# RapidAI/RapidDoc

Hardware: AMD Instinct MI355X
Metric: pages/sec (layout+OCR det/rec) (higher is better)
Workload: dtype f32

## Files before the change

### rapiddoc_amd/_lib.py

```python
from __future__ import annotations

import ctypes as C
from pathlib import Path

_PKG = Path(__file__).resolve().parent
LIB_PATH = _PKG / "librapiddoc_mi355.so"
_lib = None

SYMBOLS = {
    "rd_version": (C.c_char_p, []),
    "rd_create": (C.c_void_p, [C.c_int, C.c_char_p]),
    "rd_create_error": (C.c_char_p, []),
    "rd_destroy": (None, [C.c_void_p]),
    "rd_last_error": (C.c_char_p, [C.c_void_p]),
    "rd_load_weights": (C.c_int, [C.c_void_p, C.c_void_p, C.c_size_t]),
    "rd_query_workspace": (C.c_int, [C.c_void_p, C.c_int, C.c_int, C.c_int, C.c_int, C.POINTER(C.c_size_t)]),
    "rd_det_forward": (C.c_int, [C.c_void_p, C.c_void_p, C.c_int, C.c_int, C.c_int, C.c_void_p, C.c_void_p, C.c_size_t, C.c_void_p]),
    "rd_det_forward_ex": (C.c_int, [C.c_void_p, C.c_void_p, C.c_int, C.c_int, C.c_int, C.c_void_p, C.c_int, C.c_void_p, C.c_void_p, C.c_size_t, C.c_void_p]),
    "rd_rec_forward": (C.c_int, [C.c_void_p, C.c_void_p, C.c_int, C.c_int, C.c_void_p, C.c_void_p, C.c_void_p, C.c_int, C.c_void_p, C.c_size_t, C.c_void_p]),
    "rd_rec_num_classes": (C.c_int, [C.c_void_p]),
    "rd_rec_token_dim": (C.c_int, [C.c_void_p]),
    "rd_rec_backbone_forward": (C.c_int, [C.c_void_p, C.c_void_p, C.c_int, C.c_int, C.c_void_p, C.c_void_p, C.c_size_t, C.c_void_p]),
    "rd_rec_backbone_forward_lines": (C.c_int, [C.c_void_p, C.c_void_p, C.c_int, C.c_int, C.c_void_p, C.c_void_p, C.c_void_p, C.c_size_t, C.c_void_p]),
    "rd_rec_tail_forward": (C.c_int, [C.c_void_p, C.c_void_p, C.c_int, C.c_int, C.c_int, C.c_void_p, C.c_void_p, C.c_void_p, C.c_void_p,
# ... 3 lines not shown
    "rd_formula_encoder_forward": (C.c_int, [C.c_void_p, C.c_void_p, C.c_int, C.c_int, C.c_int, C.c_int, C.c_void_p, C.c_void_p, C.c_size_t, C.c_void_p]),
    "rd_formula_decode": (C.c_int, [C.c_void_p, C.c_void_p, C.c_int, C.c_int, C.c_int, C.c_void_p, C.POINTER(C.c_int32), C.c_void_p]),
    "rd_formula_decode_stream": (C.c_int, [C.c_void_p, C.c_void_p, C.c_int, C.c_int, C.c_int, C.c_int, C.c_void_p, C.c_void_p, C.c_void_p, C.c_void_p]),
    "rd_formula_max_new_tokens": (C.c_int, [C.c_void_p]),
    "rd_preproc_resize_norm": (C.c_int, [C.c_int, C.c_void_p, C.c_int, C.c_int, C.c_int, C.c_int, C.POINTER(C.c_float), C.POINTER(C.c_float), C.c_float, C.c_int, C.c_int, C.c_void_p, C.c_void_p]),
    "rd_preproc_resize_norm_batch": (C.c_int, [C.c_int, C.c_void_p, C.c_int, C.c_int, C.c_int, C.c_int, C.c_int, C.POINTER(C.c_float), C.POINTER(C.c_float), C.c_float, C.c_int, C.c_int, C.c_void_p, C.c_void_p]),
    "rd_preproc_resize_aa_norm": (C.c_int, [C.c_int, C.c_void_p, C.c_int, C.c_int, C.c_int, C.c_int, C.POINTER(C.c_float), C.POINTER(C.c_float), C.c_int, C.c_void_p, C.c_void_p, C.c_void_p]),
    "rd_formula_margin_boxes": (C.c_int, [C.c_int, C.c_void_p, C.c_int, C.c_void_p, C.c_void_p]),
    "rd_formula_preproc_plan": (C.c_int, [C.c_int, C.c_int, C.c_void_p]),
    "rd_formula_preproc_batch": (C.c_int, [C.c_int, C.c_void_p, C.c_void_p, C.c_int, C.c_void_p, C.c_void_p, C.c_void_p]),
    "rd_crop_resize_norm_batch": (C.c_int, [C.c_int, C.c_void_p, C.c_int, C.c_int, C.c_int, C.c_void_p, C.c_int, C.c_int, C.c_int, C.POINTER(C.c_float), C.POINTER(C.c_float), C.c_float, C.c_int, C.c_void_p, C.c_void_p]),
    "rd_line_crops_batch": (C.c_int, [C.c_int, C.c_void_p, C.c_int, C.c_int, C.c_int, C.c_void_p, C.c_int, C.c_int64, C.c_void_p, C.c_int, C.c_int, C.c_int, C.c_void_p, C.c_void_p]),
    "rd_line_warp_batch": (C.c_int, [C.c_int, C.c_void_p, C.c_int, C.c_int, C.c_int, C.c_void_p, C.c_int, C.c_int64, C.c_void_p, C.c_void_p]),
    "rd_line_resize_norm_batch": (C.c_int, [C.c_int, C.c_void_p, C.c_int, C.c_void_p, C.c_int, C.c_int, C.c_int, C.c_void_p, C.c_void_p]),
    "rd_cls_forward": (C.c_int, [C.c_void_p, C.c_void_p, C.c_int, C.c_int, C.c_int, C.c_void_p, C.c_int, C.c_void_p, C.c_void_p, C.c_size_t, C.c_void_p]),
    "rd_table_encoder_forward": (C.c_int, [C.c_void_p, C.c_void_p, C.c_int, C.c_int, C.c_int, C.c_void_p, C.c_void_p, C.c_size_t, C.c_void_p]),
    "rd_table_decode": (C.c_int, [C.c_void_p, C.c_void_p, C.c_int, C.c_int, C.c_int, C.c_void_p, C.c_void_p, C.c_void_p, C.c_void_p]),
    "rd_table_decode_stream": (C.c_int, [C.c_void_p, C.c_void_p, C.c_int, C.c_int, C.c_int, C.c_int, C.c_void_p, C.c_void_p, C.c_void_p, C.c_void_p, C.c_void_p]),
    "rd_line_flip180_batch": (C.c_int, [C.c_int, C.c_void_p, C.c_int, C.c_void_p, C.c_float, C.c_void_p, C.c_void_p, C.c_void_p]),
    "rd_ctc_collapse": (C.c_int, [C.c_int, C.c_void_p, C.c_void_p, C.c_int, C.c_int, C.c_void_p, C.c_int, C.c_int, C.c_void_p, C.c_int, C.c_void_p]),
    "rd_ctc_collapse_lines": (C.c_int, [C.c_int, C.c_void_p, C.c_void_p, C.c_int, C.c_void_p, C.c_int, C.c_void_p, C.c_int, C.c_int, C.c_void_p, C.c_int, C.c_void_p, C.c_void_p,
                                        C.c_void_p]),
    "rd_db_postprocess": (C.c_int, [C.c_void_p, C.c_int, C.c_int, C.c_int, C.c_void_p, C.c_float, C.c_float, C.c_float, C.c_int, C.c_int, C.c_void_p, C.c_int, C.c_void_p, C.c_int]),
    "rd_db_boxes_workspace": (C.c_size_t, [C.c_int, C.c_int, C.c_int, C.c_int, C.c_int]),
    "rd_db_boxes_device": (C.c_int, [C.c_int, C.c_void_p, C.c_int, C.c_int, C.c_int, C.c_void_p, C.c_float, C.c_float, C.c_float, C.c_int, C.c_int,
                                     C.c_int, C.c_void_p, C.c_size_t, C.c_void_p, C.c_int, C.c_void_p, C.c_void_p]),
    "rd_rec_chunk_cost": (C.c_double, [C.c_int, C.c_int, C.c_int]),
    "rd_rec_plan_chunks": (C.c_int, [C.c_void_p, C.c_int, C.c_int, C.c_int, C.c_int, C.c_int, C.c_void_p, C.c_int, C.c_void_p]),
    "rd_rec_plan_lines": (C.c_int, [C.c_void_p, C.c_void_p] + [C.c_int] * 9 + [C.c_void_p] * 4 + [C.c_int, C.c_void_p]),
    "rd_text_boxes_order_merge": (C.c_int, [C.c_void_p, C.c_void_p, C.c_int, C.c_int, C.c_void_p, C.c_void_p]),
    "rd_ctc_rows_text": (C.c_int, [C.c_void_p, C.c_int, C.c_int, C.c_void_p, C.c_int64, C.c_void_p, C.c_void_p, C.c_void_p, C.c_void_p]),
    "rd_layout_postprocess": (C.c_int, [C.c_void_p, C.c_int, C.c_int, C.c_int, C.c_int, C.c_void_p, C.c_void_p, C.c_void_p, C.c_void_p]),
    "rd_layout_postprocess_select": (C.c_int, [C.c_void_p, C.c_int, C.c_int, C.c_int, C.c_int, C.c_void_p, C.c_void_p, C.c_void_p, C.c_void_p]),
    "rd_find_external_contours": (C.c_int, [C.c_void_p, C.c_int, C.c_int, C.c_void_p, C.c_int, C.c_void_p, C.c_int, C.c_void_p, C.c_void_p]),
    "rd_find_external_contours_none": (C.c_int, [C.c_void_p, C.c_int, C.c_int, C.c_void_p, C.c_int, C.c_void_p, C.c_int, C.c_void_p, C.c_void_p]),
    "rd_checkbox_workspace": (C.c_size_t, [C.c_int, C.c_int, C.c_int, C.c_int, C.c_int, C.c_void_p]),
    "rd_checkbox_detect_device": (C.c_int, [C.c_int, C.c_void_p, C.c_int, C.c_int, C.c_int, C.c_int, C.c_int, C.c_int, C.c_void_p, C.c_size_t, C.c_void_p,
                                            C.c_void_p, C.c_void_p]),
    "rd_checkbox_finish": (C.c_int, [C.c_void_p, C.c_int, C.c_int, C.c_int, C.c_void_p, C.c_int, C.c_void_p]),
    "rd_region_canvases_workspace": (C.c_size_t, [C.c_int, C.c_int, C.c_int]),
    "rd_region_canvases": (C.c_int, [C.c_int, C.c_void_p, C.c_int, C.c_void_p, C.c_void_p, C.c_int, C.c_int, C.c_void_p, C.c_void_p, C.c_void_p, C.c_size_t,
                                     C.c_void_p]),
    "rd_stage_pack": (C.c_int, [C.c_void_p, C.c_void_p, C.c_void_p, C.c_void_p, C.c_void_p, C.c_int, C.c_void_p, C.c_int64, C.c_int]),
    "rd_stage_canvases": (C.c_int, [C.c_int, C.c_void_p, C.c_void_p, C.c_int, C.c_void_p]),
    "rd_contour_area": (C.c_double, [C.c_void_p, C.c_int]),
    "rd_arc_length": (C.c_double, [C.c_void_p, C.c_int, C.c_int]),
    "rd_approx_poly_dp": (C.c_int, [C.c_void_p, C.c_int, C.c_double, C.c_int, C.c_void_p, C.c_void_p]),
    "rd_min_area_rect_points": (C.c_int, [C.c_void_p, C.c_int, C.c_void_p]),
    "rd_polygon_area": (C.c_double, [C.c_void_p, C.c_int]),
    "rd_polygon_intersection_area": (C.c_double, [C.c_void_p, C.c_int, C.c_void_p, C.c_int]),
    "rd_fill_poly": (C.c_int, [C.c_void_p, C.c_int, C.c_int, C.c_void_p, C.c_int, C.c_int]),
    "rd_msdeform_attn": (C.c_int, [C.c_int] + [C.c_void_p] * 6 + [C.c_int] * 7 + [C.c_void_p]),
    "rd_topk_rows": (C.c_int, [C.c_int, C.c_void_p, C.c_int, C.c_int, C.c_int, C.c_void_p, C.c_void_p, C.c_void_p]),
    "rd_encoder_layer_workspace": (C.c_size_t, [C.c_int, C.c_int, C.c_int]),
    "rd_encoder_layer": (C.c_int, [C.c_int, C.c_void_p, C.c_void_p] + [C.c_int] * 6 + [C.c_void_p] * 12 + [C.c_float, C.c_void_p, C.c_void_p, C.c_size_t, C.c_void_p]),
    "rd_set_precision": (C.c_int, [C.c_void_p, C.c_char_p]),
    "rd_range_status": (C.c_int, [C.c_void_p, C.c_void_p]),
    "rd_plan_stats": (C.c_int, [C.c_void_p, C.POINTER(C.c_uint64), C.POINTER(C.c_uint64), C.POINTER(C.c_uint64)]),
    "rd_set_profiling": (C.c_int, [C.c_void_p, C.c_int]),
    "rd_profile_json": (C.c_char_p, [C.c_void_p]),
}

_I, _P, _F = C.c_int, C.c_void_p, C.c_float
DEBUG_SYMBOLS = {
    "rd_debug_det_forward_stages": (_I, [_P, _P, _I, _I, _I, _P, _P, _P]),
    "rd_debug_cls_forward_stages": (_I, [_P, _P, _I, _I, _I, _P, _P, _P, _P]),
    "rd_debug_table_decode": (_I, [_P, _P, _I, _I, _I, _P] + [_P] * 7),
    "rd_debug_table_decode_stream": (_I, [_P, _P, _I, _I, _I, _I, _P, _P, _P, _P, _P, _P, _P, _P, _I]),
    "rd_debug_table_encoder_taps": (_I, [_P, _P, _I, _I, _I, _P, _P, _P]),
    "rd_debug_formula_decode": (_I, [_P, _P, _I, _I, _I, _P, C.POINTER(C.c_int32), _P, _P, _P]),
    "rd_debug_formula_decode_stream": (_I, [_P, _P, _I, _I, _I, _I, _P, _P, _P, _P, _P, _P, _P, _I]),
    "rd_debug_resize_aa_coeffs": (_I, [_I, _I, _P, _P, C.c_int64]),
    "rd_debug_resample_coeffs": (_I, [_I, _I, C.c_double, C.c_double, _I, _P, _P, C.c_int64]),
    "rd_debug_region_keep_mask": (_I, [_I, _I, _P, _I, _P]),
    "rd_debug_time_mixer": (_F, [_I] * 4 + [_P] * 6),
    "rd_debug_time_gemm": (_F, [_I] * 5 + [_P] * 6),
    "rd_debug_gemm_h1": (_F, [_I] * 5 + [_P, _I, _P, _P, _P, _I, _P, _I, _P]),
    "rd_debug_seqconv": (_F, [_I] * 8 + [_P, _I, _P, _I, _P, _P, _P, _P, _I, _P]),
    "rd_debug_det_local": (_F, [_I] * 5 + [_P] * 5 + [_F, _P, C.POINTER(C.c_int)]),
    "rd_debug_conv_route": (_I, [_I] * 17 + [_P, _I]),
    "rd_debug_conv_ex": (_F, [_I] * 22 + [_P] * 10 + [C.c_char_p, _P, _I, _P]),
    "rd_debug_conv": (_F, [_I] * 14 + [_P] * 8),
    "rd_debug_stem34": (_F, [_I] * 11 + [_P] * 7),
    "rd_debug_dwconv_ex": (_F, [_I] * 17 + [_P] * 10 + [_I]),
    "rd_debug_dwconv": (_F, [_I] * 8 + [_P] * 8),
    "rd_debug_dw_route": (_I, [_I] * 9 + [_P, _I, _P]),
    "rd_debug_weight_split": (_I, [_P, _I, _I, _P, _P]),
    "rd_debug_lcv3_dw": (_F, [_I] * 9 + [_P] * 8),
    "rd_debug_dw5_strip": (_F, [_I] * 11 + [_P] * 7),
    "rd_debug_mv1e_pool": (_I, [_I] * 4 + [_P] * 3),
    "rd_debug_derived_tensor": (C.c_long, [C.c_char_p, C.c_char_p, C.c_size_t, C.c_char_p, _P, C.c_long]),
    "rd_debug_mbv3_dw": (_F, [_I] * 12 + [_P] * 4),
    "rd_debug_mbv3_block": (_F, [_I] * 14 + [_P] * 8),
    "rd_debug_mbv3_block_ok": (_I, [_I] * 12),
    "rd_debug_mbv3s_dw": (_F, [_I] * 13 + [_P] * 4),
    "rd_debug_mbv3s_block": (_F, [_I] * 15 + [_P] * 12),
    "rd_debug_lcv3_dw_det": (_F, [_I] * 10 + [_P] * 5),
    "rd_debug_lcv3_block": (_F, [_I] * 9 + [_P] * 9),
    "rd_debug_time_ctc": (_F, [_I] * 4 + [_P] * 7 + [_I, _P]),
    "rd_debug_time_checkbox_mask": (_F, [_I] * 4 + [_P, _P]),
    "rd_debug_attention": (_I, [_I] * 4 + [_F, _P, _P, _P, _I, _P]),
    "rd_debug_vit_attention": (_I, [_I] * 4 + [_F, _P, _P]),
    "rd_debug_attention_limits": (_I, [_I, _P, _P]),
    "rd_debug_layernorm": (_I, [_I, _I, _P, _I, _P, _I, _P, _P, _F]),
    "rd_debug_se_chain": (_I, [_I] * 7 + [_F] + [_I] * 3 + [_P] * 9),
    "rd_debug_maxpool2x2s1": (_I, [_I] * 6 + [_P] * 2),
    "rd_debug_avgpool3x2": (_I, [_I] * 6 + [_P] * 3),
    "rd_debug_mask_cols": (_I, [_I] * 5 + [_P, _P, _I]),
    "rd_debug_upsample": (_I, [_I] * 8 + [_P] * 2),
    "rd_debug_add": (_I, [_I] * 5 + [_P] * 3),
    "rd_debug_det_head_tail": (_I, [_I] * 4 + [_P] * 6),
    "rd_debug_ctc_head": (_I, [_I] * 3 + [_P, _I] + [_P] * 6 + [_I, _P, _P]),
    "rd_debug_dec_gemv": (_I, [_I] * 4 + [_P] * 7),
    "rd_debug_dec_attention": (_I, [_I] * 4 + [_P, _P, _I, C.c_longlong] + [_P] * 5 + [_P, _I, _P, _P, _I, _P, _I]),
    "rd_debug_dec_select": (_I, [_I, _P, _I, _I, _I, _P, _I, _P, _I, _I] + [_P] * 6),
    "rd_debug_td_gemv": (_I, [_I] * 4 + [_P] * 5),
    "rd_debug_td_attention": (_I, [_I] * 4 + [_P, _P, _I, C.c_longlong, _P, _I, _P, _P, _I, _P, _I, _P, _P]),
    "rd_debug_td_select": (_I, [_I, _P, _I, _P, _I, _P, _I, _P, _P, _P, _I, _P, _P, _P, _P, _I] + [_P] * 6),
}


class NativeLibraryError(RuntimeError):
    pass


def load():
    global _lib
    if _lib is not None:
        return _lib
    if not LIB_PATH.exists():
        raise NativeLibraryError(
            f"{LIB_PATH} is missing - build it with `python -m rapiddoc_amd.build` (hipcc, gfx950). "
            "rapiddoc_amd has no CPU fallback.")
    import torch
    lib = C.CDLL(str(LIB_PATH))
    for name, (res, args) in {**SYMBOLS, **DEBUG_SYMBOLS}.items():
        fn = getattr(lib, name)
        fn.restype = res
        fn.argtypes = args
    _lib = lib
    return lib
```

### rapiddoc_amd/csrc/api_debug.cpp

```cpp
#include <algorithm>
#include <cstring>
#include <functional>
#include <string>
#include <vector>

#include "api_handle.h"
#include "builder_util.h"
#include "region_geom.h"

extern "C" {

static float rd_debug_time(int iters, const std::function<void()>& launch, const std::function<void()>& after_first = nullptr) {
    hipEvent_t e0, e1;
    (void)hipEventCreate(&e0); (void)hipEventCreate(&e1);
    launch();
    if (after_first) after_first();
    (void)hipEventRecord(e0, nullptr);
    for (int i = 0; i < iters; ++i) launch();
    (void)hipEventRecord(e1, nullptr);
    (void)hipEventSynchronize(e1);
    float ms = 0.f;
    (void)hipEventElapsedTime(&ms, e0, e1);
    (void)hipEventDestroy(e0); (void)hipEventDestroy(e1);
    return iters > 0 ? ms / iters : 0.f;
// ... 425 lines not shown
        if ((images & 8) && !deconv && rd::conv9x9_h1_shape_ok(KH, KW, Cin, Cout)) {
            p.w9_inv = rd::prepare_conv9x9_h1_weights(hw.data(), Cout, Cin, img);
            d = nullptr;
            if (!upload(img, &d)) return done(-1.f);
            p.w9 = (const uint16_t*)d;
        }
        if (range_out) {
            if (hipHostMalloc((void**)&flag, sizeof(unsigned), hipHostMallocMapped) != hipSuccess) { flag = nullptr; return done(-1.f); }
            *flag = 0;
            p.range_flag = flag;
        }
    } else if (range_out) {
        *range_out = 0;
    }
    rd::ConvRoute route = split ? rd::conv_split_route(p, ascale != nullptr) : rd::conv_f32_route(p);
    if (force) {
        if (!debug_conv_tile(force, split, &route)) return done(-1.f);
        if (split && ((unsigned long long)N * H * W * (unsigned long long)xld >= (1ull << 32) ||
                      (unsigned long long)p.Ng * (unsigned long long)((p.K + 31) & ~31) >= (1ull << 32)))
            return done(-1.f);
    }
    if (old && split && old->code == 2 && rd::conv_stream_h3_supported(p)) route = rd::CONV_STREAM;
    else if (old && split && old->code == 1 && rd::conv_direct_h3_supported(p)) route = rd::CONV_DIRECT;
    if (ln_g && route != rd::CONV_SKINNY) return done(-1.f);
    if (route_out) *route_out = route;
    float ms = -2.f;
    try {
        ms = rd_debug_time(iters, [&] { rd::launch_conv_route(route, p, nullptr); });
    } catch (const std::exception&) {
        ms = -2.f;
    }
    return done(ms);
}

float rd_debug_conv_ex(int N, int H, int W, int Cin, int Cout, int KH, int KW, int SH, int SW, int PT, int PL, int PB, int PR, int act, int xld, int yld,
                       int rld, int out_mode, int split, int images, int allow_skinny, int iters, float* x, float* w, float* bias, float* res, float* y,
                       const float* dscale, const float* dshift, const float* ln_g, const float* ln_b, const float* ascale, const char* force,
                       char* name, int name_len, int* range_out) {
    rd::ConvRoute route = rd::CONV_F32_128x128;
    debug_copy_name("", name, name_len);
    const float ms = debug_conv_run(N, H, W, Cin, Cout, KH, KW, SH, SW, PT, PL, PB, PR, act, xld, yld, rld, out_mode, split, images, allow_skinny, iters,
                                    x, w, bias, res, y, dscale, dshift, ln_g, ln_b, ascale, force, nullptr, &route, range_out);
    if (ms != -1.f) debug_copy_name(rd::conv_route_name(route), name, name_len);
    return ms;
}

float rd_debug_conv(int N, int H, int W, int Cin, int Cout, int KH, int KW, int S, int PT, int PL, int PB, int PR, int act, int iters,
                    float* x, float* w, void* wh, void* wl, float* bias, float* res, float* y, int* used_direct) {
    const DebugConvOld old{wh, wl, used_direct ? *used_direct : 0};
    const int images = old.code == 0 ? 4 : old.code == 4 ? 8 : 0;
    rd::ConvRoute route = rd::CONV_F32_128x128;
    const float ms = debug_conv_run(N, H, W, Cin, Cout, KH, KW, S, S, PT, PL, PB, PR, act, Cin, Cout, Cout, rd::OUT_NHWC, wh != nullptr, images, 0, iters, x,
                                    w, bias, res, y, nullptr, nullptr, nullptr, nullptr, nullptr, nullptr, &old, &route, nullptr);
    if (used_direct && ms != -1.f) *used_direct = debug_conv_code(route);
    return ms;
}

float rd_debug_stem34(int N, int H, int W, int Cin, int xld, int N1, int N2, int yld, int act3, int act4, int iters, float* x, float* w3, float* b3,
                      float* w4, float* b4, float* y, unsigned* range_flag) {
    if (!rd::stem34_shape_ok(Cin, N1, N2)) return -1.f;
    std::vector<float> h3((size_t)N1 * 9 * Cin), h4((size_t)N2 * N1), hb3((size_t)((N1 + 31) / 32) * 32, 0.f);
    if (hipMemcpy(h3.data(), w3, h3.size() * 4, hipMemcpyDeviceToHost) != hipSuccess) return -1.f;
    if (hipMemcpy(h4.data(), w4, h4.size() * 4, hipMemcpyDeviceToHost) != hipSuccess) return -1.f;
    if (hipMemcpy(hb3.data(), b3, (size_t)N1 * 4, hipMemcpyDeviceToHost) != hipSuccess) return -1.f;
    std::vector<uint16_t> i3, i4;
    float inv[2];
    rd::prepare_stem34_weights(h3.data(), h4.data(), Cin, N1, N2, i3, i4, inv);
    void *d3 = nullptr, *d4 = nullptr, *db3 = nullptr;
    if (hipMalloc(&d3, i3.size() * 2) != hipSuccess || hipMalloc(&d4, i4.size() * 2) != hipSuccess || hipMalloc(&db3, hb3.size() * 4) != hipSuccess) return -1.f;
    (void)hipMemcpy(d3, i3.data(), i3.size() * 2, hipMemcpyHostToDevice);
    (void)hipMemcpy(d4, i4.data(), i4.size() * 2, hipMemcpyHostToDevice);
    (void)hipMemcpy(db3, hb3.data(), hb3.size() * 4, hipMemcpyHostToDevice);
    rd::Stem34Params p{};
    p.x = x; p.xld = xld; p.N = N; p.H = H; p.W = W; p.Cin = Cin; p.y = y; p.yld = yld;
    p.OH = (H - 1) / 2 + 1; p.OW = (W - 1) / 2 + 1; p.N1 = N1; p.N2 = N2;
    p.w3 = (const uint16_t*)d3; p.w3_inv = inv[0]; p.b3 = (const float*)db3;
    p.w4 = (const uint16_t*)d4; p.w4_inv = inv[1]; p.b4 = b4;
    p.act3 = act3; p.act4 = act4; p.range_flag = range_flag;
    const float ms = rd_debug_time(iters, [&] { rd::launch_stem34(p, nullptr); });
    (void)hipFree(d3); (void)hipFree(d4); (void)hipFree(db3);
    return ms;
}

static std::string debug_dw_route_name(const rd::DwRoute& r) {
    static const char* const kernels[] = {"pixel", "lds", "kxk_lds", "col", "tiled"};
    return std::string(kernels[r.kernel]) + (r.kernel == rd::DW_PIXEL || r.kernel == rd::DW_COL ? "" : std::to_string(r.variant));
}

float rd_debug_dwconv_ex(int N, int H, int W, int C, int KH, int KW, int SH, int SW, int PT, int PL, int PB, int PR, int act, int xld, int yld, int rld,
                         int iters, float* x, float* w, float* bias, float* res, float* y, const int32_t* line_w, const int32_t* tokinfo, float* gap,
                         int* gap_chunks, char* name, int name_len) {
    if (N <= 0 || H <= 0 || W <= 0 || C <= 0 || C % 4 != 0 || KH <= 0 || KW <= 0 || SH <= 0 || SW <= 0 || PT < 0 || PL < 0 || PB < 0 || PR < 0) return -1.f;
    if (!x || !w || !y || xld < C || xld % 4 != 0 || yld < C || yld % 4 != 0 || (res && (rld < C || rld % 4 != 0))) return -1.f;
    if (H + PT + PB < KH || W + PL + PR < KW) return -1.f;
    rd::DwParams p = rd::dw_geometry(N, H, W, C, KH, KW, SH, SW, PT, PL, PB, PR);
    if (tokinfo && !(N == 1 && H == 1 && KH == 1 && SW == 1 && p.OW == W)) return -1.f;
    if (line_w && !(SW == 1 && p.OW == W)) return -1.f;
    p.x = x; p.xld = xld; p.w = w; p.bias = bias; p.y = y; p.yld = yld; p.act = act; p.res = res; p.rld = res ? rld : 0;
    p.tokinfo = tokinfo;
    if (line_w) { p.line_w = line_w; p.line_w_stride = 1; }
    p.gap_chunks = rd::dwconv_gap_chunks(p);
    p.gap_partial = p.gap_chunks > 0 ? gap : nullptr;
    const rd::DwRoute r = rd::dw_route(p, p.gap_partial != nullptr);
    if (gap_chunks) *gap_chunks = r.kernel == rd::DW_KXK_LDS ? -1 : p.gap_chunks;
    debug_copy_name(debug_dw_route_name(r).c_str(), name, name_len);
    return rd_debug_time(iters, [&] { rd::launch_dwconv(p, nullptr); });
}

float rd_debug_dwconv(int N, int H, int W, int C, int K, int SH, int act, int iters, float* x, float* w, float* bias, float* res, float* y,
                      const int32_t* line_w, float* gap, int* gap_chunks) {
    return rd_debug_dwconv_ex(N, H, W, C, K, K, SH, 1, K / 2, K / 2, K / 2, K - 1 - K / 2, act, C, C, C, iters, x, w, bias, res, y, line_w, nullptr, gap,
                              gap_chunks, nullptr, 0);
}

int rd_debug_dw_route(int N, int H, int W, int C, int K, int SH, int ragged, int has_line_w, int wants_gap, char* name, int name_len, int* gap_chunks) {
    if (N <= 0 || H <= 0 || W <= 0 || C <= 0 || K <= 0 || SH <= 0) return -1;
    static const int32_t table[1] = {};
    rd::DwParams p{};
    p.xld = p.yld = p.rld = C; p.N = N; p.H = H; p.W = W; p.C = C;
    p.KH = ragged ? 1 : K; p.KW = ragged ? 3 : K; p.SH = SH; p.SW = 1; p.PT = p.KH / 2; p.PL = p.KW / 2;
    p.OH = (H + 2 * p.PT - p.KH) / SH + 1; p.OW = W;
    const int planned = rd::dwconv_gap_chunks(p);
    if (ragged) p.tokinfo = table;
    if (has_line_w) { p.line_w = table; p.line_w_stride = 1; }
    const rd::DwRoute r = rd::dw_route(p, wants_gap != 0);
    debug_copy_name(debug_dw_route_name(r).c_str(), name, name_len);
    if (gap_chunks) *gap_chunks = r.gap_chunks;
    return planned;
}

int rd_debug_weight_split(const float* w, int n, int clamp, uint16_t* scaled, uint16_t* h3) {
    if (!w || n <= 0 || !scaled || !h3) return -1000;
    const int ex = rd::rd_pow2_exp(w, (size_t)n, clamp);
    for (int i = 0; i < n; ++i) {
        rd::rd_split_scaled(w[i], ex, scaled[2 * i], scaled[2 * i + 1]);
        rd::rd_split_2048(w[i], h3[2 * i], h3[2 * i + 1]);
    }
    return ex;
}

float rd_debug_lcv3_dw(int N, int H, int W, int C, int K, int SH, int SW, int pre_act, int iters, const float* aff, float* x, float* w, float* bias,
                       float* y, const int32_t* line_in, const int32_t* line_out, float* gap) {
    if (!rd::lcv3_dw_shape_ok(K, SH, SW, C) || !aff || (gap && !rd::lcv3_gap_shape_ok(C))) return -1.f;
    rd::Lcv3DwParams p{};
    p.x = x; p.xld = C; p.N = N; p.H = H; p.W = W; p.C = C; p.w = w; p.bias = bias; p.y = y; p.yld = C;
    p.K = K; p.SH = SH; p.SW = SW;
    p.OH = (H + 2 * (K / 2) - K) / SH + 1; p.OW = (W + 2 * (K / 2) - K) / SW + 1;
    p.pre_act = pre_act; p.pre_s = aff[0]; p.pre_b = aff[1]; p.post_s = aff[2]; p.post_b = aff[3]; p.post_act = 1;
    p.line_in = line_in; p.line_out = line_out; p.line_stride = 1;
    return rd_debug_time(iters, [&] { rd::launch_lcv3_dw(p, nullptr); },
                         [&] { if (gap) rd::launch_lcv3_gap_rows(y, C, N, p.OH, p.OW, C, gap, line_out, 1, nullptr); });
}

float rd_debug_dw5_strip(int N, int H, int W, int C, int SH, int SW, int pre_act, int post_act, int xld, int yld, int iters, const float* aff, float* x,
                         float* w, float* bias, float* y, const int32_t* line_in, const int32_t* line_out) {
    if (!aff || SH < 1 || SW < 1) return -1.f;
    rd::Lcv3DwParams p{};
    p.x = x; p.xld = xld; p.N = N; p.H = H; p.W = W; p.C = C; p.w = w; p.bias = bias; p.y = y; p.yld = yld;
    p.K = 5; p.SH = SH; p.SW = SW;
    p.OH = (H - 1) / SH + 1; p.OW = (W - 1) / SW + 1;
    p.pre_act = pre_act; p.pre_s = aff[0]; p.pre_b = aff[1]; p.post_s = aff[2]; p.post_b = aff[3]; p.post_act = post_act;
    p.line_in = line_in; p.line_out = line_out; p.line_stride = 1;
    if (!rd::dw5_strip_launch_ok(p)) return -1.f;
    return rd_debug_time(iters, [&] { (void)rd::launch_dw5_strip(p, nullptr); });
}

// ... 330 lines not shown
```

### rapiddoc_amd/csrc/kernels_stem_fused.hip

```cpp
#include <cmath>
#include <cstdlib>
#include <vector>

#include "rd_device.h"

namespace rd {

static constexpr int SF_TH = 8, SF_TW = 32;
static constexpr int SF_EH = SF_TH + 2, SF_EW = SF_TW + 2;
static constexpr int SF_AH = SF_TH + 1, SF_AW = SF_TW + 1;
static constexpr int SF_PH = 2 * SF_EH + 1, SF_PW = 2 * SF_EW + 1;
static constexpr int SF_PROW = 208;
static constexpr int SF_PATCH_FLOATS = SF_PH * SF_PROW + 16;
static constexpr int SF_NT = 512;

template <int C1>
struct SfGeom {
    static constexpr int CA = C1, NA = C1 / 2, CB = (NA + 7) / 8 * 8;
    static constexpr int K1 = 48, K2A = 4 * CA, K2B = 4 * CB;
    static constexpr int SE = CA + 4, SA = CB + 4;
    static_assert(((SE / 4) & 1) == 1 && ((SA / 4) & 1) == 1, "pixel strides must be 4 x odd floats");
    static constexpr int pad8(int k) { return ((k / 8) & 1) ? k : k + 8; }
    static constexpr int R1 = pad8(K1), R2A = pad8(K2A), R2B = pad8(K2B);
    static constexpr int W1_H = C1 * R1, W2A_H = NA * R2A, W2B_H = C1 * R2B;
// ... 4 lines not shown
    static constexpr int A_FLOATS_RAW = (SF_AH * SF_AW + 31) / 32 * 32 * SA;
    static constexpr int A_FLOATS = A_FLOATS_RAW > SF_PATCH_FLOATS ? A_FLOATS_RAW : SF_PATCH_FLOATS;
    static constexpr size_t LDS_BYTES = (size_t)W_HALFS * 2 + (size_t)(BIAS_FLOATS + E_FLOATS + A_FLOATS) * 4 + 64;
    static constexpr int MB1 = (SF_EH * SF_EW + 31) / 32, NB1 = (C1 + 31) / 32;
    static constexpr int MB2 = (SF_AH * SF_AW + 31) / 32;
    static constexpr int MB3 = SF_TH * SF_TW / 32, NB3 = (C1 + 31) / 32;
    static_assert(NA <= 32 && MB3 == 8, "one N block for stem2a, one M block per wavefront for stem2b");
};

struct StemFusedParams {
    const float* x; int N, H, W, in_ch;
    const uint16_t* wimg;
    const float* bias;
    float* y; int yld;
    int H2, W2, tiles_x, tiles_y;
    unsigned* range_flag;
    const int32_t* line_tab;
    int dbg;
};

typedef _Float16 sf_f16x2 __attribute__((ext_vector_type(2)));
__device__ __forceinline__ void sf_split8(const f32x4 a, const f32x4 b, float neg1, f16x8& hi, f16x8& lo) {
#pragma unroll
    for (int e = 0; e < 4; e += 2) {
        const sf_f16x2 ha = __builtin_convertvector(f32x2{a[e], a[e + 1]}, sf_f16x2);
        const sf_f16x2 hb = __builtin_convertvector(f32x2{b[e], b[e + 1]}, sf_f16x2);
        hi[e] = ha[0];
        hi[e + 1] = ha[1];
        hi[4 + e] = hb[0];
        hi[4 + e + 1] = hb[1];
        lo[e] = (_Float16)__builtin_fmaf((float)ha[0], neg1, a[e]);
        lo[e + 1] = (_Float16)__builtin_fmaf((float)ha[1], neg1, a[e + 1]);
        lo[4 + e] = (_Float16)__builtin_fmaf((float)hb[0], neg1, b[e]);
        lo[4 + e + 1] = (_Float16)__builtin_fmaf((float)hb[1], neg1, b[e + 1]);
    }
}

template <int C1>
__global__ void __launch_bounds__(SF_NT, 2) stem_fused_kernel(StemFusedParams p) {
    using G = SfGeom<C1>;
    extern __shared__ __attribute__((aligned(16))) unsigned char lds[];
    _Float16* Wl = reinterpret_cast<_Float16*>(lds);
    float* Bs = reinterpret_cast<float*>(lds + (size_t)G::W_HALFS * 2);
    float* Es = Bs + ((G::BIAS_FLOATS + 3) & ~3);
    float* As = Es + G::E_FLOATS;
    const _Float16* W1h = Wl;
    const _Float16* W1l = Wl + G::W1_H;
    const _Float16* W2Ah = Wl + 2 * G::W1_H;
    const _Float16* W2Al = W2Ah + G::W2A_H;
    const _Float16* W2Bh = W2Ah + 2 * G::W2A_H;
    const _Float16* W2Bl = W2Bh + G::W2B_H;
    const float* b1 = Bs;
    const float* b2a = Bs + C1;
    const float* b2b = Bs + C1 + G::NA;

    const int tid = threadIdx.x, lane = tid & 63;
    const int wave = __builtin_amdgcn_readfirstlane(tid >> 6);
    const int l31 = lane & 31, lhi = lane >> 5;
    const float* scl = reinterpret_cast<const float*>(p.wimg + G::W_HALFS);
    const float inv1 = scl[0], inv2a = scl[1], inv2b = scl[2], sc1 = scl[3], sc2a = scl[4], sc2b = scl[5];
    float neg1 = -1.f;
    asm volatile("" : "+s"(neg1));

    for (int i = tid; i < G::W_HALFS / 8; i += SF_NT)
        reinterpret_cast<u32x4*>(Wl)[i] = reinterpret_cast<const u32x4*>(p.wimg)[i];
    for (int i = tid; i < G::BIAS_FLOATS; i += SF_NT) Bs[i] = p.bias[i];

    const int tiles_per_img = p.tiles_x * p.tiles_y, ntiles = p.N * tiles_per_img;
    constexpr int PATCH_ELEMS = SF_PH * SF_PW * 3;
    constexpr int PRE = (PATCH_ELEMS + SF_NT - 1) / SF_NT;
    float pre[PRE];
    auto tile_origin = [&](int t, int& n, int& ty0, int& tx0) {
        n = t / tiles_per_img;
        const int r = t - n * tiles_per_img;
        const int tyi = r / p.tiles_x;
        ty0 = tyi * SF_TH;
        tx0 = (r - tyi * p.tiles_x) * SF_TW;
    };
    int p_rc[PRE], p_lds[PRE], p_ci[PRE];
#pragma unroll
    for (int k = 0; k < PRE; ++k) {
        const int i = tid + k * SF_NT;
        const int row = i / (SF_PW * 3), rem = i - row * (SF_PW * 3);
        const int col = rem / 3, ci = rem - col * 3;
        p_rc[k] = i < PATCH_ELEMS ? (row << 16) | col : -1;
        p_lds[k] = row * SF_PROW + rem;
        p_ci[k] = (p.in_ch == 1 ? 0 : ci) * p.H * p.W;
    }
    auto load_patch = [&](int t) {
        int n, ty0, tx0;
        tile_origin(t, n, ty0, tx0);
        const int iy0 = 2 * ty0 - 1, ix0 = 2 * tx0 - 1;
        const float* img = p.x + (size_t)n * p.in_ch * p.H * p.W;
#pragma unroll
        for (int k = 0; k < PRE; ++k) {
            const int iy = min(max(iy0 + (p_rc[k] >> 16), 0), p.H - 1), ix = min(max(ix0 + (p_rc[k] & 0xffff), 0), p.W - 1);
            pre[k] = img[p_ci[k] + iy * p.W + ix];
        }
    };
    auto store_patch = [&](int ty0, int tx0) {
        const int iy0 = 2 * ty0 - 1, ix0 = 2 * tx0 - 1;
#pragma unroll
        for (int k = 0; k < PRE; ++k) {
            const int iy = iy0 + (p_rc[k] >> 16), ix = ix0 + (p_rc[k] & 0xffff);
            const bool ok = (unsigned)iy < (unsigned)p.H && (unsigned)ix < (unsigned)p.W;
            if (p_rc[k] >= 0) As[p_lds[k]] = ok ? pre[k] : 0.f;
        }
        if (tid < SF_PH) As[tid * SF_PROW + SF_PW * 3] = 0.f;
        if (tid >= 64 && tid < 80) As[SF_PH * SF_PROW + tid - 64] = 0.f;
    };

    unsigned emax = 0;
    int t = blockIdx.x;
    if (t < ntiles) load_patch(t);
    __syncthreads();
    for (; t < ntiles; t += gridDim.x) {
        int n, ty0, tx0;
        tile_origin(t, n, ty0, tx0);
        if (!(p.dbg & 16)) store_patch(ty0, tx0);
        __syncthreads();

        const int W2n = p.line_tab ? min(p.W2, p.line_tab[n * kLineTabStride + 1]) : p.W2;
        const bool inner = ty0 + SF_EH <= p.H2 && tx0 + SF_EW <= W2n;

        for (int mb = wave; mb < G::MB1 && !(p.dbg & 1); mb += 8) {
            const int m = min(mb * 32 + l31, SF_EH * SF_EW - 1);
            const int ey = m / SF_EW, ex = m - ey * SF_EW;
            f32x16 acc1[G::NB1], acc2[G::NB1];
#pragma unroll
            for (int nb = 0; nb < G::NB1; ++nb) {
                const float bv = b1[min(nb * 32 + l31, C1 - 1)] * sc1;
#pragma unroll
                for (int r = 0; r < 16; ++r) { acc1[nb][r] = bv; acc2[nb][r] = 0.f; }
            }
            const float* src0 = As + 2 * ey * SF_PROW + 2 * ex * 3 + 8 * lhi;
            f32x2 q[4];
            f16x8 wh[G::NB1], wl[G::NB1];
            auto fetch1 = [&](int kh) {
                const float* src = src0 + kh * SF_PROW;
#pragma unroll
                for (int i = 0; i < 4; ++i) q[i] = *reinterpret_cast<const f32x2*>(src + 2 * i);
#pragma unroll
                for (int nb = 0; nb < G::NB1; ++nb) {
                    const _Float16* wb = W1h + min(nb * 32 + l31, C1 - 1) * G::R1 + 8 * lhi + kh * 16;
                    wh[nb] = *reinterpret_cast<const f16x8*>(wb);
                    wl[nb] = *reinterpret_cast<const f16x8*>(wb + G::W1_H);
                }
            };
            fetch1(0);
#pragma unroll
            for (int kh = 0; kh < 3; ++kh) {
                const f32x4 v0 = f32x4{q[0][0], q[0][1], q[1][0], q[1][1]}, v1 = f32x4{q[2][0], q[2][1], q[3][0], q[3][1]};
                f16x8 bh[G::NB1], bl[G::NB1];
#pragma unroll
                for (int nb = 0; nb < G::NB1; ++nb) { bh[nb] = wh[nb]; bl[nb] = wl[nb]; }
                f16x8 ah, al;
                sf_split8(v0, v1, neg1, ah, al);
                __builtin_amdgcn_sched_barrier(0);
                if (kh + 1 < 3) fetch1(kh + 1);
                __builtin_amdgcn_sched_barrier(0);
#pragma unroll
                for (int nb = 0; nb < G::NB1; ++nb) {
                    acc1[nb] = __builtin_amdgcn_mfma_f32_32x32x16_f16(ah, bh[nb], acc1[nb], 0, 0, 0);
                    acc2[nb] = __builtin_amdgcn_mfma_f32_32x32x16_f16(ah, bl[nb], acc2[nb], 0, 0, 0);
                    acc2[nb] = __builtin_amdgcn_mfma_f32_32x32x16_f16(al, bh[nb], acc2[nb], 0, 0, 0);
                }
                __builtin_amdgcn_sched_barrier(0);
            }
#pragma unroll
            for (int nb = 0; nb < G::NB1; ++nb) {
                const int nn = nb * 32 + l31;
                float* dst = Es + (mb * 32 + 4 * lhi) * G::SE + nn;
                if (nn < C1) {
#pragma unroll
                    for (int r = 0; r < 16; ++r)
                        dst[((r & 3) + 8 * (r >> 2)) * G::SE] = fmaxf((acc1[nb][r] + acc2[nb][r]) * inv1, 0.f);
                }
            }
        }
        __syncthreads();
        const int vh = p.H2 - ty0, vw = W2n - tx0;
        if (!inner) {
            constexpr int C4 = C1 / 4;
            for (int i = tid; i < SF_EH * SF_EW * C4; i += SF_NT) {
                const int pix = i / C4, cg = i - pix * C4;
                const int cy = pix / SF_EW, cx = pix - cy * SF_EW;
                if (cy >= vh || cx >= vw) *reinterpret_cast<f32x4*>(Es + pix * G::SE + 4 * cg) = f32x4{0.f, 0.f, 0.f, 0.f};
            }
            __syncthreads();
        }

        for (int mb = wave; mb < G::MB2 && !(p.dbg & 2); mb += 8) {
            const int m = min(mb * 32 + l31, SF_AH * SF_AW - 1);
            const int ay = m / SF_AW, ax = m - ay * SF_AW;
            const int nrow = min(l31, G::NA - 1);
            const float bv = b2a[nrow] * sc2a;
            f32x16 acc1, acc2;
#pragma unroll
            for (int r = 0; r < 16; ++r) { acc1[r] = bv; acc2[r] = 0.f; }
            const float* src0 = Es + (ay * SF_EW + ax) * G::SE;
            const _Float16* wb = W2Ah + nrow * G::R2A + 8 * lhi;
            f32x4 nv0, nv1;
            f16x8 nbh, nbl;
            auto fetch2a = [&](int j) {
                constexpr int CAc = G::CA;
                const int t0 = (16 * j) / CAc, c0 = (16 * j) % CAc, t1 = (16 * j + 8) / CAc, c1 = (16 * j + 8) % CAc;
                const int o0 = ((t0 >> 1) * SF_EW + (t0 & 1)) * G::SE + c0, o1 = ((t1 >> 1) * SF_EW + (t1 & 1)) * G::SE + c1;
                const float* src = src0 + (lhi ? o1 : o0);
                nv0 = *reinterpret_cast<const f32x4*>(src);
                nv1 = *reinterpret_cast<const f32x4*>(src + 4);
                nbh = *reinterpret_cast<const f16x8*>(wb + 16 * j);
                nbl = *reinterpret_cast<const f16x8*>(wb + G::W2A_H + 16 * j);
            };
            fetch2a(0);
#pragma unroll
            for (int j = 0; j < G::K2A / 16; ++j) {
                const f32x4 v0 = nv0, v1 = nv1;
                const f16x8 bh = nbh, bl = nbl;
                f16x8 ah, al;
                sf_split8(v0, v1, neg1, ah, al);
                __builtin_amdgcn_sched_barrier(0);
                if (j + 1 < G::K2A / 16) fetch2a(j + 1);
                __builtin_amdgcn_sched_barrier(0);
                acc1 = __builtin_amdgcn_mfma_f32_32x32x16_f16(ah, bh, acc1, 0, 0, 0);
                acc2 = __builtin_amdgcn_mfma_f32_32x32x16_f16(ah, bl, acc2, 0, 0, 0);
                acc2 = __builtin_amdgcn_mfma_f32_32x32x16_f16(al, bh, acc2, 0, 0, 0);
                __builtin_amdgcn_sched_barrier(0);
            }
            float* dst = As + (mb * 32 + 4 * lhi) * G::SA + l31;
            const bool lane_on = l31 < G::CB;
            const bool real = l31 < G::NA;
            if (lane_on) {
#pragma unroll
                for (int r = 0; r < 16; ++r) {
                    const float v = (acc1[r] + acc2[r]) * inv2a;
                    dst[((r & 3) + 8 * (r >> 2)) * G::SA] = real ? fmaxf(v, 0.f) : 0.f;
                }
            }
        }
        {
            constexpr int C4 = C1 / 4;
            constexpr int FIRST = G::MB2 > 8 ? G::MB2 - 8 : 0, NTH = (8 - FIRST) * 64;
            if (wave >= FIRST && !(p.dbg & 4)) {
                for (int i = tid - FIRST * 64; i < SF_TH * SF_TW * C4; i += NTH) {
                    const int pix = i / C4, cg = i - pix * C4;
                    const int py = pix >> 5, px = pix & 31;
                    const int gy = ty0 + py, gx = tx0 + px;
                    if (gy >= p.H2 || gx >= p.W2) continue;
                    const float* e0 = Es + (py * SF_EW + px) * G::SE + 4 * cg;
                    const f32x4 a = *reinterpret_cast<const f32x4*>(e0), b = *reinterpret_cast<const f32x4*>(e0 + G::SE);
                    const f32x4 c = *reinterpret_cast<const f32x4*>(e0 + SF_EW * G::SE), d = *reinterpret_cast<const f32x4*>(e0 + (SF_EW + 1) * G::SE);
                    f32x4 o;
#pragma unroll
                    for (int k = 0; k < 4; ++k) o[k] = fmaxf(fmaxf(a[k], b[k]), fmaxf(c[k], d[k]));
                    emax = max(emax, __float_as_uint(o[0] + o[1] + o[2] + o[3]) & 0x7fffffffu);
                    __builtin_nontemporal_store(o, reinterpret_cast<f32x4*>(p.y + (((size_t)n * p.H2 + gy) * p.W2 + gx) * p.yld + 4 * cg));
                }
            }
        }
        __syncthreads();
        if (!inner) {
            constexpr int B4 = G::CB / 4;
            for (int i = tid; i < SF_AH * SF_AW * B4; i += SF_NT) {
                const int pix = i / B4, cg = i - pix * B4;
                const int ay = pix / SF_AW, ax = pix - ay * SF_AW;
                if (ay >= vh || ax >= vw) *reinterpret_cast<f32x4*>(As + pix * G::SA + 4 * cg) = f32x4{0.f, 0.f, 0.f, 0.f};
            }
            __syncthreads();
        }

        const int tn = t + (int)gridDim.x;
        if (tn < ntiles && !(p.dbg & 16)) load_patch(tn);

        if (!(p.dbg & 8)) {
            const int by = wave, bx = l31;
            f32x16 acc1[G::NB3], acc2[G::NB3];
#pragma unroll
            for (int nb = 0; nb < G::NB3; ++nb) {
                const float bv = b2b[min(nb * 32 + l31, C1 - 1)] * sc2b;
#pragma unroll
                for (int r = 0; r < 16; ++r) { acc1[nb][r] = bv; acc2[nb][r] = 0.f; }
            }
            const float* src0 = As + (by * SF_AW + bx) * G::SA;
            f32x4 nv0, nv1;
            f16x8 nwh[G::NB3], nwl[G::NB3];
            auto fetch2b = [&](int j) {
                constexpr int CBc = G::CB;
                const int t0 = (16 * j) / CBc, c0 = (16 * j) % CBc, t1 = (16 * j + 8) / CBc, c1 = (16 * j + 8) % CBc;
                const int o0 = ((t0 >> 1) * SF_AW + (t0 & 1)) * G::SA + c0, o1 = ((t1 >> 1) * SF_AW + (t1 & 1)) * G::SA + c1;
                const float* src = src0 + (lhi ? o1 : o0);
                nv0 = *reinterpret_cast<const f32x4*>(src);
                nv1 = *reinterpret_cast<const f32x4*>(src + 4);
#pragma unroll
                for (int nb = 0; nb < G::NB3; ++nb) {
                    const int nrow = min(nb * 32 + l31, C1 - 1);
                    nwh[nb] = *reinterpret_cast<const f16x8*>(W2Bh + nrow * G::R2B + 16 * j + 8 * lhi);
                    nwl[nb] = *reinterpret_cast<const f16x8*>(W2Bl + nrow * G::R2B + 16 * j + 8 * lhi);
                }
            };
            fetch2b(0);
#pragma unroll
            for (int j = 0; j < G::K2B / 16; ++j) {
                const f32x4 v0 = nv0, v1 = nv1;
                f16x8 bh[G::NB3], bl[G::NB3];
#pragma unroll
                for (int nb = 0; nb < G::NB3; ++nb) { bh[nb] = nwh[nb]; bl[nb] = nwl[nb]; }
                f16x8 ah, al;
                sf_split8(v0, v1, neg1, ah, al);
                __builtin_amdgcn_sched_barrier(0);
                if (j + 1 < G::K2B / 16) fetch2b(j + 1);
                __builtin_amdgcn_sched_barrier(0);
#pragma unroll
                for (int nb = 0; nb < G::NB3; ++nb) {
                    acc1[nb] = __builtin_amdgcn_mfma_f32_32x32x16_f16(ah, bh[nb], acc1[nb], 0, 0, 0);
                    acc2[nb] = __builtin_amdgcn_mfma_f32_32x32x16_f16(ah, bl[nb], acc2[nb], 0, 0, 0);
                    acc2[nb] = __builtin_amdgcn_mfma_f32_32x32x16_f16(al, bh[nb], acc2[nb], 0, 0, 0);
                }
                __builtin_amdgcn_sched_barrier(0);
            }
            __builtin_amdgcn_s_waitcnt(0x0F70);
            const int gy = ty0 + by;
            float* yrow = p.y + (((size_t)n * p.H2 + min(gy, p.H2 - 1)) * p.W2 + tx0 + 4 * lhi) * p.yld + C1;
#pragma unroll
            for (int nb = 0; nb < G::NB3; ++nb) {
                const int nn = nb * 32 + l31;
                if (inner) {
                    if (nn < C1) {
#pragma unroll
                        for (int r = 0; r < 16; ++r) {
                            const float v = (acc1[nb][r] + acc2[nb][r]) * inv2b;
                            emax = max(emax, __float_as_uint(v) & 0x7fffffffu);
                            __builtin_nontemporal_store(fmaxf(v, 0.f), &yrow[(size_t)((r & 3) + 8 * (r >> 2)) * p.yld + nn]);
                        }
                    }
                } else {
#pragma unroll
                    for (int r = 0; r < 16; ++r) {
                        const int off = (r & 3) + 8 * (r >> 2);
                        const float v = (acc1[nb][r] + acc2[nb][r]) * inv2b;
                        emax = max(emax, __float_as_uint(v) & 0x7fffffffu);
                        if (gy < p.H2 && tx0 + 4 * lhi + off < p.W2 && nn < C1)
                            yrow[(size_t)off * p.yld + nn] = tx0 + 4 * lhi + off < W2n ? fmaxf(v, 0.f) : 0.f;
                    }
                }
            }
        }
        __syncthreads();
    }
    if (emax >= 0x7f800000u && p.range_flag) rd_raise_flag(p.range_flag);
}

bool stem_fused_supported(int c1) { return c1 == 24 || c1 == 32 || c1 == 48; }

template <int C1>
static void sf_prepare(const float* w1, const float* w2a, const float* w2b, std::vector<uint16_t>& img) {
    using G = SfGeom<C1>;
    img.assign(G::IMG_HALFS, 0);
    const int ex[3] = {rd_pow2_exp(w1, (size_t)27 * C1, RD_EXP_CLAMP), rd_pow2_exp(w2a, (size_t)G::NA * G::K2A, RD_EXP_CLAMP),
                       rd_pow2_exp(w2b, (size_t)C1 * 4 * G::NA, RD_EXP_CLAMP)};
    auto put = [&](size_t hi_at, size_t lo_at, float v, int e) { rd_split_scaled(v, e, img[hi_at], img[lo_at]); };
    for (int co = 0; co < C1; ++co)
        for (int kh = 0; kh < 3; ++kh)
            for (int j = 0; j < 9; ++j)
                put((size_t)co * G::R1 + kh * 16 + j, (size_t)G::W1_H + (size_t)co * G::R1 + kh * 16 + j, w1[(size_t)(kh * 9 + j) * C1 + co], ex[0]);
    const size_t o2a = 2 * (size_t)G::W1_H;
    for (int n = 0; n < G::NA; ++n)
        for (int k = 0; k < G::K2A; ++k)
            put(o2a + (size_t)n * G::R2A + k, o2a + G::W2A_H + (size_t)n * G::R2A + k, w2a[(size_t)n * G::K2A + k], ex[1]);
    const size_t o2b = o2a + 2 * (size_t)G::W2A_H;
    for (int n = 0; n < C1; ++n)
        for (int tap = 0; tap < 4; ++tap)
            for (int c = 0; c < G::NA; ++c)
                put(o2b + (size_t)n * G::R2B + tap * G::CB + c, o2b + G::W2B_H + (size_t)n * G::R2B + tap * G::CB + c,
                    w2b[(size_t)n * 4 * G::NA + tap * G::NA + c], ex[2]);
    float scl[6];
    for (int k = 0; k < 3; ++k) { scl[k] = std::ldexp(1.f, -ex[k]); scl[3 + k] = std::ldexp(1.f, ex[k]); }
    __builtin_memcpy(&img[G::W_HALFS], scl, sizeof(scl));
}
void prepare_stem_fused_weights(int c1, const float* w1, const float* w2a, const float* w2b, std::vector<uint16_t>& img) {
    if (c1 == 24) sf_prepare<24>(w1, w2a, w2b, img);
    else if (c1 == 32) sf_prepare<32>(w1, w2a, w2b, img);
    else sf_prepare<48>(w1, w2a, w2b, img);
}

template <int C1>
static void sf_launch(StemFusedParams& p, hipStream_t s, int n_cu) {
    static unsigned long long lds_ok = 0;
    rd_allow_dynamic_lds((const void*)stem_fused_kernel<C1>, SfGeom<C1>::LDS_BYTES, lds_ok);
    const int ntiles = p.N * p.tiles_x * p.tiles_y;
    hipLaunchKernelGGL(stem_fused_kernel<C1>, dim3(ntiles < n_cu ? ntiles : n_cu), dim3(SF_NT), SfGeom<C1>::LDS_BYTES, s, p);
}

void launch_stem_fused(int c1, const float* x, int N, int H, int W, int in_ch, const uint16_t* wimg, const float* bias, float* y, int yld,
                       unsigned* range_flag, hipStream_t s, const int32_t* line_tab) {
    const int n_cu = rd_cu_count();
    StemFusedParams p{};
    p.x = x; p.N = N; p.H = H; p.W = W; p.in_ch = in_ch;
    p.wimg = wimg; p.bias = bias; p.y = y; p.yld = yld;
    p.H2 = (H + 2 - 3) / 2 + 1;
    p.W2 = (W + 2 - 3) / 2 + 1;
    p.tiles_y = (p.H2 + SF_TH - 1) / SF_TH;
    p.tiles_x = (p.W2 + SF_TW - 1) / SF_TW;
    p.range_flag = range_flag;
    p.line_tab = line_tab;
    static const int dbg = rd_env_int("RD_STEM_DBG", 0);
    p.dbg = dbg;
    if (c1 == 24) sf_launch<24>(p, s, n_cu);
    else if (c1 == 32) sf_launch<32>(p, s, n_cu);
    else sf_launch<48>(p, s, n_cu);
}

}
```

Before: 374.6.

## Stage fused-stem outputs through LDS for vectorized stores and column-walk maxpool

The final conv output of the fused stem kernel is now staged per wave in the shared-memory E tile, then written to global memory as coalesced 16-byte vector stores instead of scattered scalar stores. The maxpool branch walks each column down the tile and reuses the horizontal max of the previous row, so each row of E is read once instead of twice. The patch-load index mapping is changed to channel-major order so global reads are contiguous. A non-finite check on intermediate activations is added, and a debug timing entry point is exposed. This relies on reusing the E tile as scratch after the earlier stages have consumed it, which is only correct if the synchronisation there is sufficient.

```diff
diff --git a/rapiddoc_amd/_lib.py b/rapiddoc_amd/_lib.py
--- a/rapiddoc_amd/_lib.py
+++ b/rapiddoc_amd/_lib.py
@@ -109,6 +109,7 @@
     "rd_debug_conv_ex": (_F, [_I] * 22 + [_P] * 10 + [C.c_char_p, _P, _I, _P]),
     "rd_debug_conv": (_F, [_I] * 14 + [_P] * 8),
     "rd_debug_stem34": (_F, [_I] * 11 + [_P] * 7),
+    "rd_debug_stem_fused": (_F, [_I] * 7 + [_P] * 10),
     "rd_debug_dwconv_ex": (_F, [_I] * 17 + [_P] * 10 + [_I]),
     "rd_debug_dwconv": (_F, [_I] * 8 + [_P] * 8),
     "rd_debug_dw_route": (_I, [_I] * 9 + [_P, _I, _P]),
diff --git a/rapiddoc_amd/csrc/api_debug.cpp b/rapiddoc_amd/csrc/api_debug.cpp
--- a/rapiddoc_amd/csrc/api_debug.cpp
+++ b/rapiddoc_amd/csrc/api_debug.cpp
@@ -531,6 +531,30 @@
     return ms;
 }
 
+float rd_debug_stem_fused(int c1, int N, int H, int W, int in_ch, int yld, int iters, float* x, float* w1, float* w2a, float* w2b, float* b1,
+                          float* b2a, float* b2b, float* y, const int32_t* line_tab, unsigned* range_flag) {
+    if (!rd::stem_fused_supported(c1) || (in_ch != 1 && in_ch != 3) || N <= 0 || H <= 0 || W <= 0 || yld < 2 * c1) return -1.f;
+    const int na = c1 / 2;
+    std::vector<float> h1((size_t)27 * c1), h2a((size_t)na * 4 * c1), h2b((size_t)c1 * 4 * na), hb((size_t)c1 + na + c1);
+    if (hipMemcpy(h1.data(), w1, h1.size() * 4, hipMemcpyDeviceToHost) != hipSuccess) return -1.f;
+    if (hipMemcpy(h2a.data(), w2a, h2a.size() * 4, hipMemcpyDeviceToHost) != hipSuccess) return -1.f;
+    if (hipMemcpy(h2b.data(), w2b, h2b.size() * 4, hipMemcpyDeviceToHost) != hipSuccess) return -1.f;
+    if (hipMemcpy(hb.data(), b1, (size_t)c1 * 4, hipMemcpyDeviceToHost) != hipSuccess) return -1.f;
+    if (hipMemcpy(hb.data() + c1, b2a, (size_t)na * 4, hipMemcpyDeviceToHost) != hipSuccess) return -1.f;
+    if (hipMemcpy(hb.data() + c1 + na, b2b, (size_t)c1 * 4, hipMemcpyDeviceToHost) != hipSuccess) return -1.f;
+    std::vector<uint16_t> img;
+    rd::prepare_stem_fused_weights(c1, h1.data(), h2a.data(), h2b.data(), img);
+    void *dimg = nullptr, *dbias = nullptr;
+    if (hipMalloc(&dimg, img.size() * 2) != hipSuccess || hipMalloc(&dbias, hb.size() * 4) != hipSuccess) return -1.f;
+    (void)hipMemcpy(dimg, img.data(), img.size() * 2, hipMemcpyHostToDevice);
+    (void)hipMemcpy(dbias, hb.data(), hb.size() * 4, hipMemcpyHostToDevice);
+    const float ms = rd_debug_time(iters, [&] {
+        rd::launch_stem_fused(c1, x, N, H, W, in_ch, (const uint16_t*)dimg, (const float*)dbias, y, yld, range_flag, nullptr, line_tab);
+    });
+    (void)hipFree(dimg); (void)hipFree(dbias);
+    return ms;
+}
+
 static std::string debug_dw_route_name(const rd::DwRoute& r) {
     static const char* const kernels[] = {"pixel", "lds", "kxk_lds", "col", "tiled"};
     return std::string(kernels[r.kernel]) + (r.kernel == rd::DW_PIXEL || r.kernel == rd::DW_COL ? "" : std::to_string(r.variant));
diff --git a/rapiddoc_amd/csrc/kernels_stem_fused.hip b/rapiddoc_amd/csrc/kernels_stem_fused.hip
--- a/rapiddoc_amd/csrc/kernels_stem_fused.hip
+++ b/rapiddoc_amd/csrc/kernels_stem_fused.hip
@@ -110,9 +110,9 @@
     for (int k = 0; k < PRE; ++k) {
         const int i = tid + k * SF_NT;
         const int row = i / (SF_PW * 3), rem = i - row * (SF_PW * 3);
-        const int col = rem / 3, ci = rem - col * 3;
+        const int ci = rem / SF_PW, col = rem - ci * SF_PW;
         p_rc[k] = i < PATCH_ELEMS ? (row << 16) | col : -1;
-        p_lds[k] = row * SF_PROW + rem;
+        p_lds[k] = row * SF_PROW + col * 3 + ci;
         p_ci[k] = (p.in_ch == 1 ? 0 : ci) * p.H * p.W;
     }
     auto load_patch = [&](int t) {
@@ -138,6 +138,7 @@
         if (tid >= 64 && tid < 80) As[SF_PH * SF_PROW + tid - 64] = 0.f;
     };
 
+    float nonfin = 0.f;
     unsigned emax = 0;
     int t = blockIdx.x;
     if (t < ntiles) load_patch(t);
@@ -201,8 +202,11 @@
                 float* dst = Es + (mb * 32 + 4 * lhi) * G::SE + nn;
                 if (nn < C1) {
 #pragma unroll
-                    for (int r = 0; r < 16; ++r)
-                        dst[((r & 3) + 8 * (r >> 2)) * G::SE] = fmaxf((acc1[nb][r] + acc2[nb][r]) * inv1, 0.f);
+                    for (int r = 0; r < 16; ++r) {
+                        const float v = (acc1[nb][r] + acc2[nb][r]) * inv1;
+                        nonfin = __builtin_fmaf(v, 0.f, nonfin);
+                        dst[((r & 3) + 8 * (r >> 2)) * G::SE] = fmaxf(v, 0.f);
+                    }
                 }
             }
         }
@@ -262,6 +266,7 @@
 #pragma unroll
                 for (int r = 0; r < 16; ++r) {
                     const float v = (acc1[r] + acc2[r]) * inv2a;
+                    nonfin = __builtin_fmaf(v, 0.f, nonfin);
                     dst[((r & 3) + 8 * (r >> 2)) * G::SA] = real ? fmaxf(v, 0.f) : 0.f;
                 }
             }
@@ -270,19 +275,32 @@
             constexpr int C4 = C1 / 4;
             constexpr int FIRST = G::MB2 > 8 ? G::MB2 - 8 : 0, NTH = (8 - FIRST) * 64;
             if (wave >= FIRST && !(p.dbg & 4)) {
-                for (int i = tid - FIRST * 64; i < SF_TH * SF_TW * C4; i += NTH) {
-                    const int pix = i / C4, cg = i - pix * C4;
-                    const int py = pix >> 5, px = pix & 31;
-                    const int gy = ty0 + py, gx = tx0 + px;
-                    if (gy >= p.H2 || gx >= p.W2) continue;
-                    const float* e0 = Es + (py * SF_EW + px) * G::SE + 4 * cg;
-                    const f32x4 a = *reinterpret_cast<const f32x4*>(e0), b = *reinterpret_cast<const f32x4*>(e0 + G::SE);
-                    const f32x4 c = *reinterpret_cast<const f32x4*>(e0 + SF_EW * G::SE), d = *reinterpret_cast<const f32x4*>(e0 + (SF_EW + 1) * G::SE);
-                    f32x4 o;
-#pragma unroll
-                    for (int k = 0; k < 4; ++k) o[k] = fmaxf(fmaxf(a[k], b[k]), fmaxf(c[k], d[k]));
-                    emax = max(emax, __float_as_uint(o[0] + o[1] + o[2] + o[3]) & 0x7fffffffu);
-                    __builtin_nontemporal_store(o, reinterpret_cast<f32x4*>(p.y + (((size_t)n * p.H2 + gy) * p.W2 + gx) * p.yld + 4 * cg));
+                for (int i = tid - FIRST * 64; i < SF_TW * C4; i += NTH) {
+                    const int px = i / C4, cg = i - px * C4;
+                    const int gx = tx0 + px;
+                    if (gx >= p.W2) continue;
+                    const float* e0 = Es + px * G::SE + 4 * cg;
+                    float* yp = p.y + (((size_t)n * p.H2 + ty0) * p.W2 + gx) * p.yld + 4 * cg;
+                    const size_t ypitch = (size_t)p.W2 * p.yld;
+                    f32x4 h0;
+                    {
+                        const f32x4 a = *reinterpret_cast<const f32x4*>(e0), b = *reinterpret_cast<const f32x4*>(e0 + G::SE);
+#pragma unroll
+                        for (int k = 0; k < 4; ++k) h0[k] = fmaxf(a[k], b[k]);
+                    }
+#pragma unroll
+                    for (int py = 0; py < SF_TH; ++py) {
+                        const float* e1 = e0 + (py + 1) * SF_EW * G::SE;
+                        const f32x4 c = *reinterpret_cast<const f32x4*>(e1), d = *reinterpret_cast<const f32x4*>(e1 + G::SE);
+                        f32x4 h1, o;
+#pragma unroll
+                        for (int k = 0; k < 4; ++k) { h1[k] = fmaxf(c[k], d[k]); o[k] = fmaxf(h0[k], h1[k]); }
+                        h0 = h1;
+                        if (ty0 + py < p.H2) {
+                            emax = max(emax, __float_as_uint(o[0] + o[1] + o[2] + o[3]) & 0x7fffffffu);
+                            __builtin_nontemporal_store(o, reinterpret_cast<f32x4*>(yp + py * ypitch));
+                        }
+                    }
                 }
             }
         }
@@ -348,33 +366,39 @@
             }
             __builtin_amdgcn_s_waitcnt(0x0F70);
             const int gy = ty0 + by;
-            float* yrow = p.y + (((size_t)n * p.H2 + min(gy, p.H2 - 1)) * p.W2 + tx0 + 4 * lhi) * p.yld + C1;
+            float* stage = Es + wave * 32 * G::SE;
 #pragma unroll
             for (int nb = 0; nb < G::NB3; ++nb) {
                 const int nn = nb * 32 + l31;
-                if (inner) {
-                    if (nn < C1) {
-#pragma unroll
-                        for (int r = 0; r < 16; ++r) {
-                            const float v = (acc1[nb][r] + acc2[nb][r]) * inv2b;
-                            emax = max(emax, __float_as_uint(v) & 0x7fffffffu);
-                            __builtin_nontemporal_store(fmaxf(v, 0.f), &yrow[(size_t)((r & 3) + 8 * (r >> 2)) * p.yld + nn]);
-                        }
-                    }
-                } else {
+                if (nn < C1) {
 #pragma unroll
                     for (int r = 0; r < 16; ++r) {
-                        const int off = (r & 3) + 8 * (r >> 2);
                         const float v = (acc1[nb][r] + acc2[nb][r]) * inv2b;
                         emax = max(emax, __float_as_uint(v) & 0x7fffffffu);
-                        if (gy < p.H2 && tx0 + 4 * lhi + off < p.W2 && nn < C1)
-                            yrow[(size_t)off * p.yld + nn] = tx0 + 4 * lhi + off < W2n ? fmaxf(v, 0.f) : 0.f;
+                        stage[(4 * lhi + (r & 3) + 8 * (r >> 2)) * G::SE + nn] = fmaxf(v, 0.f);
+                    }
+                }
+            }
+            __builtin_amdgcn_fence(__ATOMIC_ACQ_REL, "workgroup");
+            __builtin_amdgcn_wave_barrier();
+            if (gy < p.H2) {
+                constexpr int C4 = C1 / 4;
+                static_assert(32 * C4 % 64 == 0 && 256 * G::SE <= G::E_FLOATS, "whole passes of the wavefront; eight slices inside the e tile");
+                float* yrow = p.y + (((size_t)n * p.H2 + gy) * p.W2 + tx0) * p.yld + C1;
+#pragma unroll
+                for (int i = lane; i < 32 * C4; i += 64) {
+                    const int px = i / C4, cg = i - px * C4;
+                    if (tx0 + px < p.W2) {
+                        f32x4 o = *reinterpret_cast<const f32x4*>(stage + px * G::SE + 4 * cg);
+                        if (tx0 + px >= W2n) o = f32x4{0.f, 0.f, 0.f, 0.f};
+                        __builtin_nontemporal_store(o, reinterpret_cast<f32x4*>(yrow + (size_t)px * p.yld + 4 * cg));
                     }
                 }
             }
         }
         __syncthreads();
     }
+    if (nonfin != 0.f) emax = 0x7f800000u;
     if (emax >= 0x7f800000u && p.range_flag) rd_raise_flag(p.range_flag);
 }
 
```

New measurement: 369.8. -1.3%, worse.
